# AER-RC/RRTMG_LW

Measured on AMD Instinct MI355X. Metric: columns/sec, 72-layer profiles, higher is better.
Workload: dtype f64 (transmittance / tfn codes and their LDS table f32); 1 GPU; 1000000 synthetic 72-layer columns, config 'cloudy' (icld=2: rtrnmr max-random overlap, idrv=0), sharded 1x1000000; ncol_total=1000000, nlay=72, columns_per_gpu=1000000, parallelism=columns/1, gather=none, kdata=stand-in (real k-data absent from the reference mount), sweeps=production

## Files before the change

### include/rrtmg_lw_hip.h

```cpp
#ifndef RRTMG_LW_HIP_H
#define RRTMG_LW_HIP_H

#ifdef __cplusplus
extern "C" {
#endif

#define RRTMG_LW_HIP_OK 0
#define RRTMG_LW_HIP_EPHYSICS 1
#define RRTMG_LW_HIP_EARG 2
#define RRTMG_LW_HIP_ENODEVICE 3
#define RRTMG_LW_HIP_ENOTINIT 4
#define RRTMG_LW_HIP_EDATA 5
#define RRTMG_LW_HIP_EHIP 6

#define RRTMG_LW_NBND 16
#define RRTMG_LW_NGPT 140

int rrtmg_lw_hip_init(const char *static_tables_path, const char *kdata_path, double cpdair, int device);

int rrtmg_lw_hip_init_devices(const char *static_tables_path, const char *kdata_path, double cpdair, int ndev, const int *devices);
int rrtmg_lw_hip_num_devices(void);

int rrtmg_lw_hip_kdata_is_standin(void);

// ... 208 lines not shown
    double *uflx, double *dflx, double *hr, double *uflxc, double *dflxc, double *hrc,
    double *duflx_dt, double *duflxc_dt);
int rrtmg_lw_hip_queue_flush(void);
int rrtmg_lw_hip_queue_columns(void);

unsigned rrtmg_lw_hip_build_flags(void);
int rrtmg_lw_hip_set_batch(int ncol_batch);
int rrtmg_lw_hip_effective_batch(int nlay);
int rrtmg_lw_hip_set_overlap(int on);
int rrtmg_lw_hip_set_cu_partition(int layer_cus);
int rrtmg_lw_hip_cu_partition(void);
int rrtmg_lw_hip_set_one_sweep_max(int ncol);
int rrtmg_lw_hip_set_split_max(int ncol);
int rrtmg_lw_hip_set_graph_max(int ncol);
void rrtmg_lw_hip_graph_stats(long long *captures, long long *replays);
int rrtmg_lw_hip_set_wide_window(int on);

int rrtmg_lw_hip_set_layer_split(int on);
int rrtmg_lw_hip_set_column_sort(int on, int min_gain);
int rrtmg_lw_hip_column_sort_min(void);
int rrtmg_lw_hip_set_column_sort_clear(int percent);
int rrtmg_lw_hip_column_sort_clear(void);
int rrtmg_lw_hip_set_clear_groups(int on);
long long rrtmg_lw_hip_workspace_bytes(void);
int rrtmg_lw_hip_set_n1_prototype(int on);
int rrtmg_lw_hip_n1_prototype(void);
int rrtmg_lw_hip_num_chunks(void);
int rrtmg_lw_hip_gpoints(void);

void rrtmg_lw_hip_profile_begin(void);
int rrtmg_lw_hip_profile_end(char *buf, int len);

int rrtmg_lw_hip_host_register(void *ptr, long long bytes);
int rrtmg_lw_hip_host_unregister(void *ptr);
int rrtmg_lw_hip_host_is_registered(const void *ptr, long long bytes);
int rrtmg_lw_hip_host_static(const void *ptr, long long bytes);
int rrtmg_lw_hip_host_changed(const void *ptr, int keep);
void rrtmg_lw_hip_combine_stats(long long *calls, long long *passes);

int rrtmg_lw_hip_gas_optics(int ncol, int nlay, int idrv,
    const double *play, const double *plev, const double *tlay, const double *tlev, const double *tsfc,
    const double *h2ovmr, const double *o3vmr, const double *co2vmr, const double *ch4vmr, const double *n2ovmr,
    const double *o2vmr, const double *cfc11vmr, const double *cfc12vmr, const double *cfc22vmr,
    const double *ccl4vmr, const double *emis,
    double *taug, double *fracs, double *planklay, double *planklev, double *plankbnd, double *dplankbnd_dt);
int rrtmg_lw_hip_gas_optics_device(int ncol, int nlay, int idrv,
// ... 174 lines not shown
```

### rrtmg_lw_amd/api.py

```python
from __future__ import annotations

import ctypes as C
import os

import numpy as np

_HERE = os.path.dirname(os.path.abspath(__file__))
LIB_PATH = os.environ.get("RRTMG_LW_HIP_LIB", os.path.join(_HERE, "librrtmg_lw_hip.so"))
STATIC_BLOB = os.path.join(_HERE, "data", "lw_static.bin")
STANDIN_KDATA = os.path.join(_HERE, "data", "standin.kdata.bin")
REAL_KDATA = os.path.join(os.path.dirname(_HERE), "data", "rrtmg_lw.kdata.bin")
NBND, NGPT = 16, 140

LIB_PATH_G256 = os.path.join(_HERE, "librrtmg_lw_hip_g256.so")

_dp = C.POINTER(C.c_double)
_lib = None
_libs = {}
_gpoints = 140
_initialised = False


class RrtmgLwError(RuntimeError):
    pass
# ... 164 lines not shown

def set_wide_window(on):
    return int(lib().rrtmg_lw_hip_set_wide_window(C.c_int(1 if on else 0)))


def set_column_sort(on, min_gain=-1):
    return int(lib().rrtmg_lw_hip_set_column_sort(C.c_int(1 if on else 0), C.c_int(int(min_gain))))


def column_sort_min():
    return int(lib().rrtmg_lw_hip_column_sort_min())


def set_column_sort_clear(percent):
    return int(lib().rrtmg_lw_hip_set_column_sort_clear(C.c_int(int(percent))))


def column_sort_clear():
    return int(lib().rrtmg_lw_hip_column_sort_clear())


def set_clear_groups(on):
    return int(lib().rrtmg_lw_hip_set_clear_groups(C.c_int(1 if on else 0)))


def cu_partition():
    return int(lib().rrtmg_lw_hip_cu_partition())


def _f(a, shape, dtype=np.float64):
    a = np.asfortranarray(a, dtype=dtype)
    if tuple(a.shape) != tuple(shape):
        raise ValueError(f"array has shape {a.shape}, interface declares {shape}")
    return a


def _p(a):
    return a.ctypes.data_as(_dp)


def _out_ok(a, shape, name, dtype=np.float64):
    if not (isinstance(a, np.ndarray) and a.dtype == dtype and a.flags.f_contiguous and a.flags.writeable and tuple(a.shape) == tuple(shape)):
        raise ValueError(f"output array {name!r} must be a writeable {np.dtype(dtype).name} Fortran-ordered array of shape {tuple(shape)}")
    return a


# ... 758 lines not shown
```

### rrtmg_lw_amd/csrc/driver.hip

```cpp
#include <hip/hip_runtime.h>
#include <cstdlib>
#include <sched.h>

#include <algorithm>
#include <array>
#include <atomic>
#include <cstdint>
#include <cstdarg>
#include <mutex>
#include <string>
#include <chrono>
#include <condition_variable>
#include <functional>
#include <map>
#include <thread>
#include <type_traits>
#include <vector>

#include "../../include/rrtmg_lw_hip.h"
#include "kernels.hip"
#include "mtjump.hpp"
#include "hostrows.hpp"
#include "owned.hpp"

// ... 542 lines not shown
        const State::PrepSet &ps = G.prep[0];
        W.percol = ps.percol; W.laytrop = ps.laytrop; W.ncbands = ps.ncbands; W.cflag = ps.cflag;
        W.odcld = ps.odcld; W.efcl = ps.efcl; W.ovl = ps.ovl;
        W.btop = ps.btop; W.order = ps.order; W.hgrp = ps.hgrp; W.hblk = ps.hblk; W.bbot = ps.bbot; W.hbot = ps.hbot;
    }
    G.ws = State::WsShape{nlay, ncolb, cloud, mc, want_gdp, want_efcl, want_ovl, two_scr, ng, slabcols};
    return 0;
}

int ensure_mask(int nlay, size_t ncol)
{
    const size_t bytes = (size_t)KJ_NWORD * nlay * ncol * sizeof(unsigned);
    return grow(G.mask, bytes, bytes, "sub-column masks");
}

bool g_colsort = []() { const char *e = getenv("RRTMG_LW_COLSORT"); return !e || atoi(e) != 0; }();
bool use_colsort(bool gcm, int mode, int nb);
constexpr int COLSORT_NEVER = 1 << 24;
int g_colsort_min = []() { const char *e = getenv("RRTMG_LW_COLSORT_MIN"); return e ? std::max(0, std::min(atoi(e), COLSORT_NEVER)) : 24; }();
constexpr int COLSORT_CLEAR_MAX = 1000;
constexpr int COLSORT_CLEAR_DEFAULT = 18;
int g_colsort_clear = []() { const char *e = getenv("RRTMG_LW_COLSORT_CLEAR"); return e ? std::max(0, std::min(atoi(e), COLSORT_CLEAR_MAX)) : COLSORT_CLEAR_DEFAULT; }();
bool g_clear_groups = []() { const char *e = getenv("RRTMG_LW_CLEAR_GROUPS"); return !e || atoi(e) != 0; }();

Workspace ws_for(int k, bool sorted)
{
    Workspace w = G.W;
    const State::PrepSet &ps = G.prep[k];
    w.perm = sorted ? ps.perm : nullptr;
    w.wsort = sorted ? ps.wsort : nullptr;
    w.tlayc = ps.tlayc; w.tlevc = ps.tlevc; w.cldfc = ps.cldfc;
    w.wide = ps.wide;
    w.percol = ps.percol; w.laytrop = ps.laytrop; w.ncbands = ps.ncbands; w.cflag = ps.cflag;
    w.odcld = ps.odcld; w.efcl = ps.efcl; w.ovl = ps.ovl;
    w.btop = ps.btop; w.order = ps.order; w.hgrp = ps.hgrp; w.hblk = ps.hblk; w.bbot = ps.bbot; w.hbot = ps.hbot;
    const State::ScrSet &ss = G.scrset[G.ws.two_scr ? k : 0];
    for (int a = 0; a < NSCR; a++) w.scr[a] = ss.scr[a];
    w.fw = ss.fw;
    return w;
}

int make_stream(Stream &st, int lo, int hi)
{
    if (hi <= lo) { HIP_TRY(hipStreamCreateWithFlags(st.slot(), hipStreamNonBlocking)); return 0; }
    uint32_t mask[32] = {};
    const int nw = (G.cu_total + 31) / 32;
// ... 40 lines not shown
    if (fork) HIP_TRY(hipEventRecord(G.ev_join.get(), side));
    if (scan) {
        LAUNCH("k_cloudscan", (k_cloudscan<GCM>), cgrid1, cblock1, s, Wk, g, c, b.nb, b.col0, b.nct, b.inflag, b.iceflag, b.liqflag, b.mode);
        if (fork) HIP_TRY(hipStreamWaitEvent(s, G.ev_join.get(), 0));
        const dim3 lgrid((b.nb + BLOCK - 1) / BLOCK, Wk.nlay), lblock(BLOCK);
        LAUNCH("k_cloudlay", (k_cloudlay<GCM>), lgrid, lblock, s, G.D, Wk, g, c, b.nb, b.col0, b.nct, b.mode, b.inflag, b.iceflag, b.liqflag);
        LAUNCH("k_blocksort", k_blocksort, dim3(1), dim3(256), s, Wk, (b.nb + 63) / 64, one_sweep(b.nb, b.mode) ? 1 : 0);
    }
    return launches_ok();
}

LayerArgs layer_args(const Batch &b, const double *tauaer)
{
    LayerArgs la;
    la.ncol = b.nb; la.col0 = b.col0; la.nct = b.nct; la.idrv = b.idrv; la.istart = b.istart; la.iend = b.iend;
    la.ktab_bytes = (int)(G.H.ktab.size() * 8);
    la.tauaer = tauaer;
    const unsigned gx = (b.nb + LAYER_BLOCK - 1) / LAYER_BLOCK;
    const auto bits = [](std::initializer_list<int> bands) { unsigned m = 0; for (int b : bands) m |= 1u << (b - 1); return m; };
    const unsigned quarter[4] = {bits({1, 2, 11, 15, 6}), bits({8, 10, 14, 16, 12, 13}), bits({4, 9, 7}), bits({3, 5})};
    const unsigned pairs_ = gx * (unsigned)b.nlay;
    la.nparts = !g_layer_split ? 1 : (pairs_ * 4 <= 1152 ? 4 : (pairs_ * 2 <= 1152 ? 2 : 1));
    for (int p = 0; p < 4; p++) la.partmask[p] = la.nparts == 4 ? quarter[p] : (la.nparts == 2 && p < 2 ? (quarter[2 * p] | quarter[2 * p + 1]) : 0xffffu);
    return la;
}

template <bool GCM>
int run_layer(hipStream_t s, const Workspace &Wk, const Batch &b, const GcmIn &g, const ColIn &c)
{
    const dim3 block(BLOCK);
    if (b.mode == 3) {
        const dim3 cgrid((b.nb + BLOCK - 1) / BLOCK, b.nlay);
        if (b.mc) LAUNCH("k_cloudmc<arrays>", (k_cloudmc<false>), cgrid, block, s, G.D, Wk, *b.mc, g, b.nb, b.col0, b.nct, b.inflag, b.iceflag, b.liqflag);
        else LAUNCH("k_cloudmc<mask>", (k_cloudmc<true>), cgrid, block, s, G.D, Wk, McIn{}, g, b.nb, b.col0, b.nct, b.inflag, b.iceflag, b.liqflag);
        LAUNCH("k_blocksort", k_blocksort, dim3(1), dim3(256), s, Wk, (b.nb + 63) / 64, one_sweep(b.nb, b.mode) ? 1 : 0);
    }
    const LayerArgs la = layer_args(b, GCM ? g.tauaer : c.taua);
    const unsigned gx = (b.nb + LAYER_BLOCK - 1) / LAYER_BLOCK;
    const dim3 lgrid(gx, b.nlay, la.nparts), lblock(LAYER_BLOCK);
    Workspace Wn = Wk;
    if (!GCM || !HAVE_WIDE || !g_wide_window) Wn.wide = nullptr;
    const dim3 wgrid(gx * b.nlay, la.nparts);
    if (Wn.wide) HIP_TRY(hipMemsetAsync(Wn.wide, 0, sizeof(int), s));
    if (b.share != 0) {
        if constexpr (GCM && !TUNING) {
            if (b.mode != 3 || b.mc || !Wk.odg) return fail(RRTMG_LW_HIP_EARG, "internal: shared gas optics without the mask or the optical-depth array");
            if (b.share == 1) {
                LAUNCH("k_layer<mcshare,0>", (k_layer<true, CL_SHARE, 0>), lgrid, lblock, s, G.D, Wn, g, c, la);
                if (Wn.wide) LAUNCH("k_layer<mcshare,1>", (k_layer<true, CL_SHARE, 1>), wgrid, lblock, s, G.D, Wn, g, c, la);
            } else {
                LAUNCH("k_codet", k_codet, dim3((b.nb + BLOCK - 1) / BLOCK, b.nlay), block, s, G.D, Wk, b.nb, b.col0);
            }
            return launches_ok();
        } else return fail(RRTMG_LW_HIP_EARG, "shared gas optics: GCM entries only");
    }
    const int cloud = b.mode == 0 ? 0 : b.mode == 3 ? (b.mc ? 2 : 3) : 1;
    if (TUNING && !GCM) return fail(RRTMG_LW_HIP_EARG, "tuning build: GCM entry only");
    if (TUNING && cloud != 1) return fail(RRTMG_LW_HIP_EARG, "tuning build: cloudy non-McICA calls only");
    static const char *const names[4][2] = {{"k_layer<clear,0>", "k_layer<clear,1>"}, {"k_layer<cloud,0>", "k_layer<cloud,1>"},
                                            {"k_layer<mcica,0>", "k_layer<mcica,1>"}, {"k_layer<mcmask,0>", "k_layer<mcmask,1>"}};
    if (int rc = with_const<0, 1, 2, 3>(cloud, [&](auto CL) {
            constexpr int cl = decltype(CL)::value;
// ... 140 lines not shown
    const size_t b_pc = align_up((size_t)NPERCOL * n * 8, 256), b_lt = align_up(n * 4, 256);
    const size_t b_wide = align_up((2 + ((n + LAYER_BLOCK - 1) / LAYER_BLOCK) * L) * 4, 256);
    if (int rc = grow(G.opt_buf, b_pc + b_lt + b_wide, b_pc + b_lt + b_wide, "gas-optics workspace")) return rc;
    G.opt_percol = G.opt_buf.as<double>();
    G.opt_laytrop = (int *)(G.opt_buf.as<char>() + b_pc);
    G.opt_wide = (int *)(G.opt_buf.as<char>() + b_pc + b_lt);
    HIP_TRY(hipMemset(G.opt_wide, 0, 8));
    G.opt_nlay = nlay;
    G.opt_ncolb = ncolb;
    return 0;
}

template <bool GCM>
int run_optics(hipStream_t s, const Batch &b, const GcmIn &g, const ColIn &c, const OptOut &o)
{
    Workspace W{};
    W.ncolb = G.opt_ncolb; W.pcb = G.opt_ncolb; W.nlay = b.nlay; W.err = G.d_err.as<int>();
    W.percol = G.opt_percol; W.laytrop = G.opt_laytrop;
    W.wide = GCM && HAVE_WIDE && g_wide_window ? G.opt_wide : nullptr;
    LAUNCH("k_colprep", (k_colprep<GCM>), dim3((b.nb + 63) / 64), dim3(64), s, G.D, W, g, c, b.nb, b.col0, b.nct, b.idrv, 1, 0);
    const LayerArgs la = layer_args(b, nullptr);
    const unsigned gx = (b.nb + LAYER_BLOCK - 1) / LAYER_BLOCK;
    if (W.wide) HIP_TRY(hipMemsetAsync(W.wide, 0, sizeof(int), s));
    LAUNCH("k_optics", (k_optics<GCM, 0>), dim3(gx, b.nlay, la.nparts), dim3(LAYER_BLOCK), s, G.D, W, g, c, la, o);
    if constexpr (GCM && HAVE_WIDE) {
        if (W.wide) LAUNCH("k_optics<wide>", (k_optics<true, 1>), dim3(gx * b.nlay, la.nparts), dim3(LAYER_BLOCK), s, G.D, W, g, c, la, o);
    }
    return launches_ok();
}

int check_optics(int idrv, const OptOut &o)
{
    if (!o.taug || !o.fracs) return fail(RRTMG_LW_HIP_EARG, "gas optics: taug and fracs are required");
    if (idrv == 1 && !o.dplankbnd) return fail(RRTMG_LW_HIP_EARG, "gas optics: idrv=1 needs dplankbnd_dt");
    return 0;
}

int ensure_pipeline()
{
    if (G.aux) return 0;
    Event *const ev[] = {&G.ev_in, &G.ev_last, &G.ev_fork, &G.ev_join, &G.ev_ready[0], &G.ev_layer[0], &G.ev_done[0], &G.ev_ready[1], &G.ev_layer[1], &G.ev_done[1]};
    int rc = 0;
    for (Event *e : ev) if (rc == 0) rc = make_event(*e);
    if (rc == 0) rc = make_stream(G.aux, 0, 0);
    if (rc != 0) for (Event *e : ev) (void)e->reset();
    return rc;
}
// ... 22 lines not shown
    const McIn *const mc = call.mc;
    const int nbmax = balanced_batch(ncol, eff_batch(nlay));
    const bool single = ncol <= nbmax && !(G.split_sweep && G.cu_layer > 0);
    const hipStream_t aux = single ? s : G.aux.get();
    ColIn c{};
    const bool split = G.split_sweep && G.ws.two_scr && !(mode == 3 && mc);
    const bool part = split && G.cu_layer > 0;
    if (part && !G.lay_m) {
        if (int rc = make_stream(G.lay_u, 0, 0)) return rc;
        if (int rc = make_stream(G.lay_m, 0, G.cu_layer)) return rc;
    }
    if (G.ev_last_valid) HIP_TRY(hipStreamWaitEvent(s, G.ev_last.get(), 0));
    State::GraphEnt *gent = nullptr;
    bool capture = false;
    if (single && !split && !gen.on && !mc && !G.profile && !G.n1 && ncol <= g_graph_max) {
        std::vector<unsigned char> key;
        key_put(key, ncol); key_put(key, call.nct); key_put(key, nlay); key_put(key, mode); key_put(key, idrv); key_put(key, call.inflag); key_put(key, call.iceflag); key_put(key, call.liqflag);
        const double *gp[] = {g.play, g.plev, g.tlay, g.tlev, g.tsfc, g.h2ovmr, g.o3vmr, g.co2vmr, g.ch4vmr, g.n2ovmr, g.o2vmr, g.cfc11vmr, g.cfc12vmr,
                              g.cfc22vmr, g.ccl4vmr, g.emis, g.cldfr, g.taucld, g.cicewp, g.cliqwp, g.reice, g.reliq, g.tauaer, g.tauctot,
                              out.uflx, out.dflx, out.hr, out.uflxc, out.dflxc, out.hrc, out.duflx_dt, out.duflxc_dt, out.fnet, out.fnetc,
                              out.uflxs, out.dflxs, out.uflxcs, out.dflxcs, out.uflx_var, out.dflx_var, out.hr_var};
        key_put(key, gp);
        key_put(key, G.init_gen); key_put(key, G.device);
        key_put(key, G.ws_buf.get()); key_put(key, G.ws_buf.bytes()); key_put(key, g_colsort); key_put(key, g_colsort_min); key_put(key, g_colsort_clear); key_put(key, g_clear_groups); key_put(key, g_one_sweep_max);
        key_put(key, g_wide_window); key_put(key, g_layer_split); key_put(key, g_prep_fork); key_put(key, G.sweep_fanout); key_put(key, eff_batch(nlay)); key_put(key, g_split_max);
        for (auto &e : G.graphs) if (e.key == key) { gent = &e; break; }
        if (!gent) {
            if (G.graphs.size() >= GRAPH_CACHE) {
                size_t old = 0;
                for (size_t j = 1; j < G.graphs.size(); j++) if (G.graphs[j].used < G.graphs[old].used) old = j;
                G.graphs.erase(G.graphs.begin() + (long)old);
            }
            G.graphs.emplace_back();
            gent = &G.graphs.back();
            gent->key = key;
        }
        gent->used = ++G.graph_clock;
        if (gent->exec) {
            HIP_TRY(hipGraphLaunch(gent->exec.get(), s));
            G.graph_replays++;
            HIP_TRY(hipEventRecord(G.ev_last.get(), s));
            G.ev_last_valid = true;
            return 0;
        }
        capture = gent->seen >= 1 && !gent->failed;
        gent->seen++;
        if (capture && !G.cap) { if (int rc = make_stream(G.cap, 0, 0)) return rc; }
// ... 1228 lines not shown
}

int rrtmg_lw_hip_set_column_sort_clear(int percent)
{
    ENTRY_LOCK;
    const int prev = g_colsort_clear;
    g_colsort_clear = std::max(0, std::min(percent, COLSORT_CLEAR_MAX));
    return prev;
}
int rrtmg_lw_hip_column_sort_clear(void)
{
    ENTRY_LOCK;
    return g_colsort_clear;
}

int rrtmg_lw_hip_set_clear_groups(int on)
{
    ENTRY_LOCK;
    const int prev = g_clear_groups ? 1 : 0;
    g_clear_groups = on != 0;
    return prev;
}

int rrtmg_lw_hip_set_cu_partition(int layer_cus)
{
    ENTRY_LOCK;
    if (!G.init) return fail(RRTMG_LW_HIP_ENOTINIT, "rrtmg_lw_hip_init has not been called");
    State *const keep = g_cur;
    int rc = 0;
    for (int d = 0; d < g_ndev && rc == 0; d++) {
        g_cur = &g_states[d];
        (void)hipSetDevice(G.device);
        (void)hipDeviceSynchronize();
        int n = layer_cus <= 0 ? 0 : std::max(8, std::min(G.cu_total - 8, (layer_cus + 4) / 8 * 8));
        if (G.cu_total < 16) n = 0;
        G.swset[1] = {};
        G.lay_u.reset();
        G.lay_m.reset();
        G.cu_layer = n;
        if (n > 0) {
            G.split_sweep = true;
            if ((rc = make_stream(G.lay_u, 0, 0)) == 0 && (rc = make_stream(G.lay_m, 0, n)) == 0) rc = ensure_sweep_set(1);
            if (rc != 0 && d > 0) g_states[0].err = G.err;
        }
    }
    g_cur = keep;
// ... 2091 lines not shown
```

### rrtmg_lw_amd/csrc/kernels.hip

```cpp
#include <hip/hip_runtime.h>
#include "kissjump.hpp"

#ifdef RRLW_TUNE
#define RRLW_BF_TUNE 1u
#else
#define RRLW_BF_TUNE 0u
#endif
#ifdef RRLW_G256
#define RRLW_BF_G256 8u
#else
#define RRLW_BF_G256 0u
#endif
#if defined(RRLW_LAYER_BLOCK) || defined(RRLW_STAGE_DOUBLES) || defined(RRLW_LAYER_WAVES) || defined(RRLW_LOAD_CHUNK) || defined(RRLW_MINOR_WIN) || \
    defined(RRLW_COLSORT_WIN) || defined(RRLW_SWEEPC_P0) || defined(RRLW_SWEEPC_P2D) || defined(RRLW_SWEEPC_WAVES_CAP) || defined(RRLW_SWEEPC_CODES) || \
    defined(RRLW_SWEEPZ_WAVES_G1) || defined(RRLW_SWEEPZ_WAVES_IDRV) || defined(RRLW_LAYER_STAMPS) || \
    defined(RRLW_DBG_DUMP)
#define RRLW_BF_GEOMETRY 16u
#else
#define RRLW_BF_GEOMETRY 0u
#endif

#include <algorithm>
#include <type_traits>
#include <utility>
// ... 3 lines not shown
namespace rrlw {

constexpr unsigned BUILD_FLAGS = RRLW_BF_TUNE | RRLW_BF_G256 | RRLW_BF_GEOMETRY;

struct DevTables {
    const double *ktab;
    const double *stat;
    BandLayout band[NBND];
    StaticLayout sl;
    double absice0[2], abscld1, absliq0;
    double delwave[NBND];
    double refrat[NBND][6];
    double heatfac, fluxfac, oneminus, bpade;
};

enum Field {
    F_FAC00, F_FAC01, F_FAC10, F_FAC11,
    F_COLH2O, F_COLCO2, F_COLO3, F_COLN2O, F_COLCO, F_COLCH4, F_COLO2, F_COLBRD,
    F_COLDRY, F_SELFFAC, F_SELFFRAC, F_FORFAC, F_FORFRAC, F_MINORFRAC, F_SCALEMINOR, F_SCALEMINORN2,
    F_PAVEL, F_WX1, F_WX2, F_WX3, F_WX4,
    NFIELD
};
enum PerCol { PC_PLANKBND = 0, PC_DPLANKBND = 16, PC_SECDIFF = 32, NPERCOL = 48 };
enum Scr { S_CODE, S_CODET, NSCR };
struct alignas(16) Part2 { double a, b; };

typedef float scr_t;
constexpr int CODE_WORDS = 4;
constexpr int CODE_BYTES = 4 * CODE_WORDS;

struct Workspace {
    int ncolb;
    int nlay;
    double *percol;
    int *laytrop;
    int *ncbands;
    double *odcld;
    double *efcl;
    int *cflag;
    double2 *ovl;
    int *btop;
    int *order;
    int *hgrp;
    int *hblk;
    int *bbot;
    int *hbot;
// ... 578 lines not shown
    R1(K_BINARY, H2O, CO2, R_H2OCO2, true, true, 0, false, 0, {NOM, NOM, NOM}, 0, {0, 0}, C_NONE, 0),
    ZERO_REGION)
BAND_TRAITS(13, 4,
    R1(K_BINARY, H2O, N2O, R_H2ON2O, true, true, 0, false, 2,
       {{A_ADJ, CO2, true, 2, 3.0, 2.0, 0.68, 3.55e-4}, {A_COL, CO, true, 4, 0, 0, 0, 0}, NOM}, 0, {0, 0}, C_NONE, 0),
    R1(K_NONE, 0, 0, 0, false, false, -1, false, 1, {{A_COL, O3, false, 0, 0, 0, 0, 0}, NOM, NOM}, 0, {0, 0}, C_NONE, 0))
BAND_TRAITS(14, 2,
    R1(K_SINGLE, CO2, 0, 0, true, true, -1, false, 0, {NOM, NOM, NOM}, 0, {0, 0}, C_NONE, 0),
    R1(K_SINGLE, CO2, 0, 0, false, false, -1, false, 0, {NOM, NOM, NOM}, 0, {0, 0}, C_NONE, 0))
BAND_TRAITS(15, 2,
    R1(K_BINARY, N2O, CO2, R_N2OCO2, true, true, 0, false, 1, {{A_BRD, BRD, true, 2, 0, 0, 0, 0}, NOM, NOM}, 0, {0, 0}, C_NONE, 0),
    ZERO_REGION)
BAND_TRAITS(16, 2,
    R1(K_BINARY, H2O, CH4, R_H2OCH4, true, true, 0, false, 0, {NOM, NOM, NOM}, 0, {0, 0}, C_NONE, 0),
    R1(K_SINGLE, CH4, 0, 0, false, false, -1, false, 0, {NOM, NOM, NOM}, 0, {0, 0}, C_NONE, 0))
#undef R1

__device__ const double kMult4[16] = {1, 1, 1, 1, 1, 1, 1, 0.92, 0.88, 1.07, 1.1, 0.99, 0.88, 0.943, 1, 1};
__device__ const double kMult7[16] = {1, 1, 1, 1, 1, 0.92, 0.88, 1.07, 1.1, 0.99, 0.855, 1, 1, 1, 1, 1};

struct LayerCoef {
    double f[NFIELD];
    int jp, jt, jt1, indself, indfor, indminor;
};

struct Spec { double speccomb, specparm, fs; int js; };
__device__ __forceinline__ Spec spec_calc(double cola, double rat, double colb, double mult, double oneminus)
{
    Spec s;
    s.speccomb = cola + rat * colb;
    s.specparm = fdiv(cola, s.speccomb);
    if (s.specparm >= oneminus) s.specparm = oneminus;
    const double specmult = mult * s.specparm;
    s.js = 1 + (int)specmult;
    s.fs = specmult - (double)(int)specmult;
    return s;
}

__device__ __forceinline__ void stencil6(double specparm, double fs, double fa, double fb, int &off, double (&w)[6])
{
    if (specparm < 0.125) {
        const double p = fs - 1, p2 = p * p, p4 = p2 * p2;
        const double fk0 = p4, fk1 = 1 - p - 2.0 * p4, fk2 = p + p4;
        off = 0;
        w[0] = fk0 * fa; w[1] = fk1 * fa; w[2] = fk2 * fa; w[3] = fk0 * fb; w[4] = fk1 * fb; w[5] = fk2 * fb;
    } else if (specparm > 0.875) {
// ... 33 lines not shown
#ifdef RRLW_G256
__host__ __device__ constexpr int band_ng(int B) { return B >= 1 ? 16 : 16; }
#else
__host__ __device__ constexpr int band_ng(int B) { return B == 1 ? 10 : B == 2 ? 12 : B == 3 ? 16 : B == 4 ? 14 : B == 5 ? 16 : B == 6 ? 8 : B == 7 ? 12 :
                                                    B == 8 ? 8 : B == 9 ? 12 : B == 10 ? 6 : B == 11 ? 8 : B == 12 ? 8 : B == 13 ? 4 : 2; }
#endif
__host__ __device__ constexpr int band_nquad(int B) { return (band_ng(B) + 3) / 4; }
__host__ __device__ constexpr int band_qstart(int B)
{
    int s = 0;
    for (int b = 1; b < B; b++) s += band_nquad(b);
    return s;
}
constexpr int NQUAD = band_qstart(17);
__host__ __device__ constexpr int band_g0(int B)
{
    int s = 0;
    for (int b = 1; b < B; b++) s += band_ng(b);
    return s;
}
static_assert(band_g0(17) == NGPT, "g-point table");
static_assert(NQUAD == (NGPT == 140 ? 38 : 64), "quad table");

constexpr int NRATCHI = 6 * 59 + 7 * 59;
__shared__ double s_ratchi[NRATCHI];

template <int N>
struct Rows {
    unsigned off[N > 0 ? N : 1];
    double w[N > 0 ? N : 1];
    unsigned fw;
};

template <int B> constexpr unsigned lo_binary_mask() { return (BT<B>::lo.key == K_BINARY ? 1u << (B - 1) : 0u) | lo_binary_mask<B - 1>(); }
template <> constexpr unsigned lo_binary_mask<0>() { return 0u; }
template <int B> constexpr unsigned up_binary_mask() { return (BT<B>::up.key == K_BINARY ? 1u << (B - 1) : 0u) | up_binary_mask<B - 1>(); }
template <> constexpr unsigned up_binary_mask<0>() { return 0u; }
template <int B> constexpr unsigned up_zero_mask() { return (BT<B>::up.key == K_ZERO ? 1u << (B - 1) : 0u) | up_zero_mask<B - 1>(); }
template <> constexpr unsigned up_zero_mask<0>() { return 0u; }
template <int B> constexpr unsigned up_from_a_mask() { return (BT<B>::up.frac_from_a ? 1u << (B - 1) : 0u) | up_from_a_mask<B - 1>(); }
template <> constexpr unsigned up_from_a_mask<0>() { return 0u; }
constexpr unsigned LO_BINARY = lo_binary_mask<16>(), UP_BINARY = up_binary_mask<16>(), UP_ZERO = up_zero_mask<16>(), UP_FROM_A = up_from_a_mask<16>();
static_assert((UP_BINARY & ~LO_BINARY) == 0u, "fw slots are assigned by the lower region");
__host__ __device__ constexpr int popcnt_c(unsigned v) { int n = 0; for (; v; v &= v - 1) n++; return n; }
constexpr int NFW = popcnt_c(LO_BINARY);
__host__ __device__ constexpr int fw_slot(int B) { return popcnt_c(LO_BINARY & ((1u << (B - 1)) - 1u)); }

template <int B, bool LOWER, int N, int IM>
__device__ __forceinline__ void rows_prep_minor(const DevTables &T, const LayerCoef &C, Rows<N> &rw)
{
    constexpr Region R = LOWER ? BT<B>::lo : BT<B>::up;
    constexpr unsigned ng = BT<B>::ng;
    constexpr Minor M = R.m[IM];
    constexpr int I0 = region_minor_base(R, LOWER, IM);
    const BandLayout &L = T.band[B - 1];
    const double mf = C.f[F_MINORFRAC];
    double amount;
    if constexpr (M.amt == A_COL) amount = C.f[F_COLH2O + M.sp];
    else if constexpr (M.amt == A_BRD_N2) amount = C.f[F_COLBRD] * C.f[F_SCALEMINORN2];
    else if constexpr (M.amt == A_O2) amount = C.f[F_COLO2] * C.f[F_SCALEMINOR];
    else if constexpr (M.amt == A_BRD) amount = C.f[F_COLBRD] * C.f[F_SCALEMINOR];
    else {
        const double colx = C.f[F_COLH2O + M.sp], coldry = C.f[F_COLDRY];
        const double chiref = M.chiconst > 0. ? M.chiconst : s_ratchi[(T.sl.chi - T.sl.rat) + M.sp * 59 + C.jp];
        const double chi = fdiv(colx, coldry);
        const double ratx = fdiv(1.e20 * chi, chiref);
        amount = colx;
        if (ratx > M.thr) amount = (M.base + pow(ratx - M.base, M.expo)) * chiref * coldry * 1.e-20;
    }
    const unsigned slot = (unsigned)(LOWER ? L.minor_lo[IM] : L.minor_up[IM]);
    if constexpr (M.two_d) {
        constexpr unsigned nj = LOWER ? 9 : 5;
        const Spec sm = spec_calc(C.f[F_COLH2O + R.a], T.refrat[B - 1][M.refslot], C.f[F_COLH2O + R.b], LOWER ? 8. : 4., T.oneminus);
        const unsigned r = slot + ((unsigned)(C.indminor - 1) * nj + (unsigned)(sm.js - 1)) * ng;
        rw.off[I0] = r;                    rw.w[I0] = amount * ((1. - mf) * (1. - sm.fs));
        rw.off[I0 + 1] = r + ng;           rw.w[I0 + 1] = amount * ((1. - mf) * sm.fs);
        rw.off[I0 + 2] = r + nj * ng;      rw.w[I0 + 2] = amount * (mf * (1. - sm.fs));
        rw.off[I0 + 3] = r + nj * ng + ng; rw.w[I0 + 3] = amount * (mf * sm.fs);
    } else {
        const unsigned r = slot + (unsigned)(C.indminor - 1) * ng;
        rw.off[I0] = r;          rw.w[I0] = amount * (1. - mf);
        rw.off[I0 + 1] = r + ng; rw.w[I0 + 1] = amount * mf;
    }
}

template <int B, bool LOWER, int N>
__device__ __forceinline__ void rows_prep(const DevTables &T, const LayerCoef &C, Rows<N> &rw)
{
    constexpr Region R = LOWER ? BT<B>::lo : BT<B>::up;
    constexpr unsigned ng = BT<B>::ng;
    const BandLayout &L = T.band[B - 1];
    const int jp = C.jp, jt = C.jt, jt1 = C.jt1;
    const double *rat_tab = s_ratchi;
    rw.fw = 0u;
    if constexpr (R.key == K_ZERO) return;

    double corradj = 1.;
    if constexpr (R.corr == C_B1LO) { if (C.f[F_PAVEL] < 250.) corradj = 1. - 0.15 * (250. - C.f[F_PAVEL]) / 154.4; }
    else if constexpr (R.corr == C_B1UP) corradj = 1. - 0.15 * (C.f[F_PAVEL] / 95.6);
    else if constexpr (R.corr == C_B2LO) corradj = 1. - .05 * (C.f[F_PAVEL] - 100.) / 900.;

    if constexpr (R.key == K_SINGLE) {
        const unsigned r0 = LOWER ? ((jp - 1) * 5 + (jt - 1)) : ((jp - 13) * 5 + (jt - 1));
        const unsigned r1 = LOWER ? (jp * 5 + (jt1 - 1)) : ((jp - 12) * 5 + (jt1 - 1));
        const unsigned tab = (unsigned)(LOWER ? L.absa : L.absb);
        const double colk = C.f[F_COLH2O + R.a];
        rw.off[0] = tab + r0 * ng;       rw.w[0] = colk * C.f[F_FAC00];
        rw.off[1] = tab + (r0 + 1) * ng; rw.w[1] = colk * C.f[F_FAC10];
        rw.off[2] = tab + r1 * ng;       rw.w[2] = colk * C.f[F_FAC01];
        rw.off[3] = tab + (r1 + 1) * ng; rw.w[3] = colk * C.f[F_FAC11];
    } else if constexpr (R.key == K_BINARY) {
        const double cola = C.f[F_COLH2O + R.a], colb = C.f[F_COLH2O + R.b];
        const double rat = rat_tab[R.rat * 59 + (jp - 1)], rat_1 = rat_tab[R.rat * 59 + jp];
        constexpr double mult = LOWER ? 8. : 4.;
        const Spec s = spec_calc(cola, rat, colb, mult, T.oneminus);
        const Spec s1 = spec_calc(cola, rat_1, colb, mult, T.oneminus);
        if constexpr (LOWER) {
            const unsigned tab = (unsigned)L.absa;
            const int ind0 = ((jp - 1) * 5 + (jt - 1)) * 9 + s.js - 1;
            const int ind1 = (jp * 5 + (jt1 - 1)) * 9 + s1.js - 1;
            int so;
            double w6[6];
            stencil6(s.specparm, s.fs, C.f[F_FAC00], C.f[F_FAC10], so, w6);
            unsigned r = tab + (unsigned)(ind0 + so) * ng;
            rw.off[0] = r;           rw.w[0] = s.speccomb * w6[0];
            rw.off[1] = r + ng;      rw.w[1] = s.speccomb * w6[1];
            rw.off[2] = r + 2 * ng;  rw.w[2] = s.speccomb * w6[2];
            rw.off[3] = r + 9 * ng;  rw.w[3] = s.speccomb * w6[3];
            rw.off[4] = r + 10 * ng; rw.w[4] = s.speccomb * w6[4];
            rw.off[5] = r + 11 * ng; rw.w[5] = s.speccomb * w6[5];
            stencil6(s1.specparm, s1.fs, C.f[F_FAC01], C.f[F_FAC11], so, w6);
            r = tab + (unsigned)(ind1 + so) * ng;
            rw.off[6] = r;            rw.w[6] = s1.speccomb * w6[0];
            rw.off[7] = r + ng;       rw.w[7] = s1.speccomb * w6[1];
            rw.off[8] = r + 2 * ng;   rw.w[8] = s1.speccomb * w6[2];
            rw.off[9] = r + 9 * ng;   rw.w[9] = s1.speccomb * w6[3];
// ... 289 lines not shown
    constexpr int NP = 4 * band_nquad(B);
    constexpr bool SCALED = BL::R.mult != 0;
#pragma unroll
    for (int j = 0; j < NP; j++) tau[j] = (SCALED || j >= BL::ng) ? 0.0 : tau0;
    if constexpr (BL::NL > 0) {
        double2 b0[BL::CH], b1[BL::CH];
        BL::template issue<0, LDS>(kt, lds, rw, b0);
        BL::template step<0, LDS>(kt, lds, rw, b0, b1, tau);
    }
    if constexpr (SCALED) {
#pragma unroll
        for (int j = 0; j < BL::ng; j++) {
            if constexpr (BL::R.mult == 4) tau[j] = fma(tau[j], kMult4[j], tau0);
            else if constexpr (BL::R.mult == 7) tau[j] = fma(tau[j], kMult7[j], tau0);
        }
    }
}

struct LayerArgs {
    int ncol, col0, nct, idrv, istart, iend;
    int nparts;
    unsigned partmask[4];
    int ktab_bytes;
    const double *tauaer;
};

struct alignas(16) scr4 { scr_t v[4]; };

typedef float scr_vec __attribute__((ext_vector_type(4)));
struct pk4 { unsigned w[CODE_WORDS]; };
__device__ __forceinline__ pk4 pack4(const scr4 &v)
{
    pk4 p;
#pragma unroll
    for (int k = 0; k < 4; k++) p.w[k] = __float_as_uint(v.v[k]);
    return p;
}
__device__ __forceinline__ scr4 unpack4(const pk4 &p)
{
    scr4 v;
#pragma unroll
    for (int k = 0; k < 4; k++) v.v[k] = __uint_as_float(p.w[k]);
    return v;
}
typedef unsigned pk_vec __attribute__((ext_vector_type(CODE_WORDS)));
__device__ __forceinline__ void scr_store(unsigned *base, size_t cell, const scr4 &v)
// ... 267 lines not shown
        }
    }
}

#ifndef RRLW_LAYER_WAVES
#define RRLW_LAYER_WAVES 3
#endif

struct LayerWg { double2 *lds; int jp0, im0, tid, nth, pc; bool lower, ok; };

template <int B, int CLOUD, class WN, int BASE_LO, int BASE_UP>
__device__ __forceinline__ void layer_band(const DevTables &T, const Workspace &W, const LayerArgs &a, const LayerCoef &C,
                                           __amdgpu_buffer_rsrc_t kt, const LayerWg &wg, bool lower, int lay, int col, bool incol, int cloudy,
                                           const unsigned (&mw)[MASK_WORDS])
{
    STAMP(4);
    unsigned delta[NROLE];
#pragma unroll
    for (int r = 0; r < NROLE; r++) delta[r] = 0u;
    const bool use_lds = __builtin_amdgcn_ballot_w64(!wg.ok) == 0ull;
    const size_t ncb = W.ncolb, gcx = (size_t)a.col0 + wg.pc;
    double odcld = 0.0;
    if constexpr (CLOUD == 1 || CLOUD == 3 || CLOUD == CL_SHARE) { if (cloudy) odcld = W.odcld[((size_t)(B - 1) * W.nlay + (lay - 1)) * ncb + col]; }
    const double secdiff = W.percol[(size_t)(PC_SECDIFF + B - 1) * ncb + col];
    const double taua = col_load(a.tauaer + (size_t)a.col0 + (size_t)a.nct * ((lay - 1) + (size_t)W.nlay * (B - 1)), (unsigned)wg.pc * 8u);
    unsigned gbits = 0u;
    if constexpr (CLOUD == 3 || CLOUD == CL_SHARE) {
        (void)mw;
        constexpr int g0 = band_g0(B), ng = BT<B>::ng, w0 = g0 >> 5, w1 = (g0 + ng - 1) >> 5;
        if (cloudy) {
            const unsigned *mrow = W.mask + (size_t)(lay - 1) * W.mask_stride + W.mask_col0 + gcx;
            const unsigned long long lo = mrow[(size_t)w0 * W.nlay * W.mask_stride];
            const unsigned long long hi = w1 != w0 ? mrow[(size_t)w1 * W.nlay * W.mask_stride] : 0u;
            gbits = (unsigned)(((lo | (hi << 32)) >> (g0 & 31)) & ((1ull << ng) - 1ull));
        }
    }
    if (lower) {
        constexpr int N = region_nrows(BT<B>::lo, true);
        Rows<N> rw;
        rows_prep<B, true, N>(T, C, rw);
        if (use_lds) {
            band_delta<B, true, WN, BASE_LO>(T, wg.jp0, wg.im0, delta);
            rows_to_lds<B, true, N>(rw, delta);
            STAMP(2);
            band_cells<B, CLOUD, true, N, true>(T, W, kt, wg.lds, rw, lay, col, incol, secdiff, taua, cloudy, odcld, gbits);
        } else {
            band_cells<B, CLOUD, true, N, false>(T, W, kt, wg.lds, rw, lay, col, incol, secdiff, taua, cloudy, odcld, gbits);
// ... 201 lines not shown
        const double tz_up = GCM ? col_load(g.tlev + ro + nct, o8) : c.tz[gc + (size_t)nct * lay];
        const double tz_lo = lay == 1 ? (GCM ? col_load(g.tlev + ro, o8) : c.tz[gc]) : 0.0;
        for (int b = 0; b < NBND; b++) {
            if (!((bmask >> b) & 1u)) continue;
            const double *tp = S + T.sl.totplnk + 181 * b;
            if (o.planklay) opt_store(o.planklay + ro + (size_t)nct * nlv * b, bytes, off8, planck_band(tp, tavel));
            if (o.planklev) {
                const size_t lv0 = (size_t)a.col0 + (size_t)nct * (nlv + 1) * b;
                opt_store(o.planklev + lv0 + (size_t)nct * lay, bytes, off8, planck_band(tp, tz_up));
                if (lay == 1) opt_store(o.planklev + lv0, bytes, off8, planck_band(tp, tz_lo));
            }
            if (lay == 1) {
                if (o.plankbnd) opt_store(o.plankbnd + a.col0 + (size_t)nct * b, bytes, off8, W.percol[(size_t)(PC_PLANKBND + b) * W.ncolb + col]);
                if (o.dplankbnd && a.idrv == 1) opt_store(o.dplankbnd + a.col0 + (size_t)nct * b, bytes, off8, W.percol[(size_t)(PC_DPLANKBND + b) * W.ncolb + col]);
            }
        }
    }
    const __amdgpu_buffer_rsrc_t kt = __builtin_amdgcn_make_buffer_rsrc((void *)T.ktab, 0, a.ktab_bytes, 0x00020000);
    const unsigned mw[MASK_WORDS] = {};
#ifdef RRLW_LAYER_STAMPS
    if ((threadIdx.x & 63) == 0) { for (int i = 0; i < NSTAMP; i++) s_stamp[(threadIdx.x >> 6) * (NSTAMP + 1) + i] = 0ull; }
    STAMP(-1);
#endif
    for (int i = threadIdx.x; i < NRATCHI; i += LAYER_BLOCK) s_ratchi[i] = S[T.sl.rat + i];
    if (!early) {
        if (threadIdx.x == 0) { s_wg[0] = lower ? 1 : 0; s_wg[1] = 99; s_wg[2] = 99; s_wg[3] = 0; s_wg[4] = 0; }
        __syncthreads();
    }
    LayerWg wg;
    wg.lds = s_tab; wg.tid = threadIdx.x; wg.nth = blockDim.x; wg.pc = pc;
    wg.lower = s_wg[0] != 0;
    if (!early) {
        const bool in = lower == wg.lower;
        int jlo = in ? jp : 99, ilo = in ? indminor : 99, jhi = in ? jp : 0, ihi = in ? indminor : 0;
#pragma unroll
        for (int o = 32; o >= 1; o >>= 1) {
            jlo = min(jlo, __shfl_xor(jlo, o, 64)); ilo = min(ilo, __shfl_xor(ilo, o, 64));
            jhi = max(jhi, __shfl_xor(jhi, o, 64)); ihi = max(ihi, __shfl_xor(ihi, o, 64));
        }
        if ((threadIdx.x & 63) == 0) { atomicMin(&s_wg[1], jlo); atomicMin(&s_wg[2], ilo); atomicMax(&s_wg[3], jhi); atomicMax(&s_wg[4], ihi); }
    }
    __syncthreads();
    wg.jp0 = s_wg[1];
    using WN = std::conditional_t<WIDE != 0, WinWide, WinNarrow>;
    wg.im0 = min(s_wg[2], 20 - WN::MW);
    wg.ok = lower == wg.lower && (unsigned)(jp - wg.jp0) <= (unsigned)(WN::NPL - 2) && (unsigned)(indminor - wg.im0) <= (unsigned)(WN::MW - 2);
    STAMP(5);
    passes_run<CLOUD, WN>(static_cast<std::conditional_t<WIDE != 0, LayerPassesWide, LayerPasses> *>(nullptr), T, W, a, C, kt, wg, lower, lay, col, incol, cloudy, mw, bmask, o);
#ifdef RRLW_LAYER_STAMPS
    STAMP(4);
    if ((threadIdx.x & 63) == 0) {
        for (int i = 0; i < NSTAMP; i++) atomicAdd(&g_stamps[i], s_stamp[(threadIdx.x >> 6) * (NSTAMP + 1) + i]);
        atomicAdd(&g_stamps[NSTAMP], 1ull);
    }
#endif
}

template <bool GCM, int CLOUD, int WIDE>
__device__ __forceinline__ void layer_grid(const DevTables &T, const Workspace &W, const GcmIn &g, const ColIn &c, const LayerArgs &a, double2 *s_tab, int *s_wg,
                                           const OptOut &o)
{
    const int part = WIDE == 0 ? blockIdx.z : blockIdx.y;
    unsigned bmask = ((a.iend >= 32 ? 0u : (1u << a.iend)) - 1u) & ~((1u << (a.istart - 1)) - 1u);
    if (a.nparts > 1) bmask &= a.partmask[part];
    if constexpr (WIDE == 0) {
        layer_cells<GCM, CLOUD, 0>(T, W, g, c, a, s_tab, s_wg, blockIdx.x, blockIdx.y, bmask, part == 0, o);
    } else {
        const int n = __builtin_amdgcn_readfirstlane(W.wide[0]), gx = (a.ncol + LAYER_BLOCK - 1) / LAYER_BLOCK;
        if ((int)blockIdx.x >= n) return;
        const int item = __builtin_amdgcn_readfirstlane(W.wide[2 + blockIdx.x]);
        layer_cells<GCM, CLOUD, 1>(T, W, g, c, a, s_tab, s_wg, item % gx, item / gx, bmask, false, o);
    }
}
template <bool GCM, int CLOUD, int WIDE>
__global__ __launch_bounds__(LAYER_BLOCK, RRLW_LAYER_WAVES) void k_layer(DevTables T, Workspace W, GcmIn g, ColIn c, LayerArgs a)
{
    __shared__ double2 s_tab[STAGE_DOUBLES / 2];
    __shared__ int s_wg[5];
    layer_grid<GCM, CLOUD, WIDE>(T, W, g, c, a, s_tab, s_wg, OptOut{});
}
template <bool GCM, int WIDE>
__global__ __launch_bounds__(LAYER_BLOCK, RRLW_LAYER_WAVES) void k_optics(DevTables T, Workspace W, GcmIn g, ColIn c, LayerArgs a, OptOut o)
{
    __shared__ double2 s_tab[STAGE_DOUBLES / 2];
    __shared__ int s_wg[5];
    layer_grid<GCM, CL_OPTICS, WIDE>(T, W, g, c, a, s_tab, s_wg, o);
}

__global__ __launch_bounds__(256) void k_codet(DevTables T, Workspace W, int ncol, int col0)
// ... 95 lines not shown
        const double factor = (radice - 2.) / 3.;
        index_i = (int)factor; if (index_i == 43) index_i = 42;
        fint_i = factor - (double)index_i;
        index_i = clampi(index_i, 1, 42);
    } else if (iceflag == 3) {
        if (radice < 5.0 || radice > 140.0) ice_err = E_ICE_GEN_BOUNDS;
        const double factor = (radice - 2.) / 3.;
        index_i = (int)factor; if (index_i == 46) index_i = 45;
        fint_i = factor - (double)index_i;
        index_i = clampi(index_i, 1, 45);
    }
    if (liqflag == 1) {
        if (radliq < 2.5 || radliq > 60.) liq_err = E_LIQ_BOUNDS;
        index_l = (int)(radliq - 1.5);
        if (index_l == 0) index_l = 1;
        if (index_l == 58) index_l = 57;
        fint_l = radliq - 1.5 - (double)index_l;
        index_l = clampi(index_l, 1, 57);
    }
    int err = 0, any = 0, quad = 0;
#pragma unroll 1
    for (int B = 1; B <= NBND; B++) {
        const int ng = band_ng(B), g0 = band_g0(B);
        const double secdiff = W.percol[(size_t)(PC_SECDIFF + B - 1) * ncb + col];
        double ai = 0.0, al = 0.0;
        if (inflag == 2) {
            if (iceflag == 0) ai = T.absice0[0] + T.absice0[1] / radice;
            else if (iceflag == 1) {
                const int icx = B <= 2 ? B : (B <= 5 ? 3 : (B <= 8 ? 4 : 5));
                ai = absice1[2 * (icx - 1)] + absice1[2 * (icx - 1) + 1] / radice;
            } else if (iceflag == 2) { const double *t = absice2 + 43 * (B - 1); ai = t[index_i - 1] + fint_i * (t[index_i] - t[index_i - 1]); }
            else if (iceflag == 3) { const double *t = absice3 + 46 * (B - 1); ai = t[index_i - 1] + fint_i * (t[index_i] - t[index_i - 1]); }
            if (liqflag == 0) al = T.absliq0;
            else if (liqflag == 1) { const double *t = absliq1 + 58 * (B - 1); al = t[index_l - 1] + fint_l * (t[index_l] - t[index_l - 1]); }
        }
        const double tband = FROMMASK ? g.taucld[(B - 1) + (size_t)NBND * cl] : 0.0;
        if constexpr (FROMMASK) {
            const unsigned long long lo = mw[g0 >> 5], hi = (g0 >> 5) < MASK_WORDS - 1 ? mw[(g0 >> 5) + 1] : 0u;
            const unsigned bits = (unsigned)(((lo | (hi << 32)) >> (g0 & 31)) & ((1ull << ng) - 1ull));
            double t = tband, od = 0.0, ef = 0.0;
            if (bits) {
                if (mciwp + mclwp >= cldmin || t >= cldmin) {
                    if (inflag == 1) err = E_MC_INFLAG1;
                    else if (inflag == 2) {
                        double a_i = 0.0, a_l = 0.0;
                        if (mciwp != 0.0 && iceflag >= 0 && iceflag <= 3) { a_i = ai; if (ice_err && !err) err = ice_err; }
                        if (mclwp != 0.0) {
// ... 2529 lines not shown
```

Before: 18.20 million columns/s.

## Shrink ratchi LDS staging to a jp window and fold constant secdiff bands

After: 17.79 million columns/s. 0.978x the previous value.

```diff
diff --git a/include/rrtmg_lw_hip.h b/include/rrtmg_lw_hip.h
--- a/include/rrtmg_lw_hip.h
+++ b/include/rrtmg_lw_hip.h
@@ -254,6 +254,7 @@
 int rrtmg_lw_hip_set_column_sort_clear(int percent);
 int rrtmg_lw_hip_column_sort_clear(void);
 int rrtmg_lw_hip_set_clear_groups(int on);
+int rrtmg_lw_hip_set_layer_order(int order);
 long long rrtmg_lw_hip_workspace_bytes(void);
 int rrtmg_lw_hip_set_n1_prototype(int on);
 int rrtmg_lw_hip_n1_prototype(void);
diff --git a/rrtmg_lw_amd/api.py b/rrtmg_lw_amd/api.py
--- a/rrtmg_lw_amd/api.py
+++ b/rrtmg_lw_amd/api.py
@@ -210,6 +210,10 @@
 
 def set_clear_groups(on):
     return int(lib().rrtmg_lw_hip_set_clear_groups(C.c_int(1 if on else 0)))
+
+
+def set_layer_order(order):
+    return int(lib().rrtmg_lw_hip_set_layer_order(C.c_int(1 if order else 0)))
 
 
 def cu_partition():
diff --git a/rrtmg_lw_amd/csrc/driver.hip b/rrtmg_lw_amd/csrc/driver.hip
--- a/rrtmg_lw_amd/csrc/driver.hip
+++ b/rrtmg_lw_amd/csrc/driver.hip
@@ -588,6 +588,8 @@
 constexpr int COLSORT_CLEAR_DEFAULT = 18;
 int g_colsort_clear = []() { const char *e = getenv("RRTMG_LW_COLSORT_CLEAR"); return e ? std::max(0, std::min(atoi(e), COLSORT_CLEAR_MAX)) : COLSORT_CLEAR_DEFAULT; }();
 bool g_clear_groups = []() { const char *e = getenv("RRTMG_LW_CLEAR_GROUPS"); return !e || atoi(e) != 0; }();
+constexpr int LAYER_ORDER_DEFAULT = 0;
+int g_layer_order = []() { const char *e = getenv("RRTMG_LW_LAYER_ORDER"); return e ? (atoi(e) != 0 ? 1 : 0) : LAYER_ORDER_DEFAULT; }();
 
 Workspace ws_for(int k, bool sorted)
 {
@@ -674,7 +676,13 @@
     const unsigned pairs_ = gx * (unsigned)b.nlay;
     la.nparts = !g_layer_split ? 1 : (pairs_ * 4 <= 1152 ? 4 : (pairs_ * 2 <= 1152 ? 2 : 1));
     for (int p = 0; p < 4; p++) la.partmask[p] = la.nparts == 4 ? quarter[p] : (la.nparts == 2 && p < 2 ? (quarter[2 * p] | quarter[2 * p + 1]) : 0xffffu);
+    la.order = g_layer_order != 0 && gx <= 65535u ? 1 : 0;
     return la;
+}
+dim3 layer_grid_dim(const LayerArgs &la, int nlay)
+{
+    const unsigned gx = (la.ncol + LAYER_BLOCK - 1) / LAYER_BLOCK;
+    return la.order ? dim3((unsigned)nlay, gx, la.nparts) : dim3(gx, (unsigned)nlay, la.nparts);
 }
 
 template <bool GCM>
@@ -689,7 +697,7 @@
     }
     const LayerArgs la = layer_args(b, GCM ? g.tauaer : c.taua);
     const unsigned gx = (b.nb + LAYER_BLOCK - 1) / LAYER_BLOCK;
-    const dim3 lgrid(gx, b.nlay, la.nparts), lblock(LAYER_BLOCK);
+    const dim3 lgrid = layer_grid_dim(la, b.nlay), lblock(LAYER_BLOCK);
     Workspace Wn = Wk;
     if (!GCM || !HAVE_WIDE || !g_wide_window) Wn.wide = nullptr;
     const dim3 wgrid(gx * b.nlay, la.nparts);
@@ -876,7 +884,7 @@
     const LayerArgs la = layer_args(b, nullptr);
     const unsigned gx = (b.nb + LAYER_BLOCK - 1) / LAYER_BLOCK;
     if (W.wide) HIP_TRY(hipMemsetAsync(W.wide, 0, sizeof(int), s));
-    LAUNCH("k_optics", (k_optics<GCM, 0>), dim3(gx, b.nlay, la.nparts), dim3(LAYER_BLOCK), s, G.D, W, g, c, la, o);
+    LAUNCH("k_optics", (k_optics<GCM, 0>), layer_grid_dim(la, b.nlay), dim3(LAYER_BLOCK), s, G.D, W, g, c, la, o);
     if constexpr (GCM && HAVE_WIDE) {
         if (W.wide) LAUNCH("k_optics<wide>", (k_optics<true, 1>), dim3(gx * b.nlay, la.nparts), dim3(LAYER_BLOCK), s, G.D, W, g, c, la, o);
     }
@@ -945,7 +953,7 @@
                               out.uflxs, out.dflxs, out.uflxcs, out.dflxcs, out.uflx_var, out.dflx_var, out.hr_var};
         key_put(key, gp);
         key_put(key, G.init_gen); key_put(key, G.device);
-        key_put(key, G.ws_buf.get()); key_put(key, G.ws_buf.bytes()); key_put(key, g_colsort); key_put(key, g_colsort_min); key_put(key, g_colsort_clear); key_put(key, g_clear_groups); key_put(key, g_one_sweep_max);
+        key_put(key, G.ws_buf.get()); key_put(key, G.ws_buf.bytes()); key_put(key, g_colsort); key_put(key, g_colsort_min); key_put(key, g_colsort_clear); key_put(key, g_clear_groups); key_put(key, g_layer_order); key_put(key, g_one_sweep_max);
         key_put(key, g_wide_window); key_put(key, g_layer_split); key_put(key, g_prep_fork); key_put(key, G.sweep_fanout); key_put(key, eff_batch(nlay)); key_put(key, g_split_max);
         for (auto &e : G.graphs) if (e.key == key) { gent = &e; break; }
         if (!gent) {
@@ -2220,6 +2228,14 @@
     return prev;
 }
 
+int rrtmg_lw_hip_set_layer_order(int order)
+{
+    ENTRY_LOCK;
+    const int prev = g_layer_order;
+    g_layer_order = order != 0 ? 1 : 0;
+    return prev;
+}
+
 int rrtmg_lw_hip_set_cu_partition(int layer_cus)
 {
     ENTRY_LOCK;
diff --git a/rrtmg_lw_amd/csrc/kernels.hip b/rrtmg_lw_amd/csrc/kernels.hip
--- a/rrtmg_lw_amd/csrc/kernels.hip
+++ b/rrtmg_lw_amd/csrc/kernels.hip
@@ -49,6 +49,8 @@
     NFIELD
 };
 enum PerCol { PC_PLANKBND = 0, PC_DPLANKBND = 16, PC_SECDIFF = 32, NPERCOL = 48 };
+__host__ __device__ constexpr bool secdiff_fixed(int B) { return B == 1 || B == 4 || B >= 10; }
+constexpr double SECDIFF_FIXED = 1.66;
 enum Scr { S_CODE, S_CODET, NSCR };
 struct alignas(16) Part2 { double a, b; };
 
@@ -673,6 +675,7 @@
 struct LayerCoef {
     double f[NFIELD];
     int jp, jt, jt1, indself, indfor, indminor;
+    int jp0, jspan;
 };
 
 struct Spec { double speccomb, specparm, fs; int js; };
@@ -752,8 +755,13 @@
 static_assert(band_g0(17) == NGPT, "g-point table");
 static_assert(NQUAD == (NGPT == 140 ? 38 : 64), "quad table");
 
-constexpr int NRATCHI = 6 * 59 + 7 * 59;
-__shared__ double s_ratchi[NRATCHI];
+constexpr int NRATCHI_TAB = 6 + 7, RATCHI_PITCH = 5;
+__shared__ double s_ratchi[NRATCHI_TAB * RATCHI_PITCH];
+__device__ __forceinline__ double ratchi(const DevTables &T, const LayerCoef &C, int tab, int d)
+{
+    const unsigned r = (unsigned)(C.jp - C.jp0);
+    return r <= (unsigned)C.jspan ? s_ratchi[tab * RATCHI_PITCH + r + d] : T.stat[T.sl.rat + tab * 59 + (C.jp - 1) + d];
+}
 
 template <int N>
 struct Rows {
@@ -792,7 +800,7 @@
     else if constexpr (M.amt == A_BRD) amount = C.f[F_COLBRD] * C.f[F_SCALEMINOR];
     else {
         const double colx = C.f[F_COLH2O + M.sp], coldry = C.f[F_COLDRY];
-        const double chiref = M.chiconst > 0. ? M.chiconst : s_ratchi[(T.sl.chi - T.sl.rat) + M.sp * 59 + C.jp];
+        const double chiref = M.chiconst > 0. ? M.chiconst : ratchi(T, C, 6 + M.sp, 1);
         const double chi = fdiv(colx, coldry);
         const double ratx = fdiv(1.e20 * chi, chiref);
         amount = colx;
@@ -821,7 +829,6 @@
     constexpr unsigned ng = BT<B>::ng;
     const BandLayout &L = T.band[B - 1];
     const int jp = C.jp, jt = C.jt, jt1 = C.jt1;
-    const double *rat_tab = s_ratchi;
     rw.fw = 0u;
     if constexpr (R.key == K_ZERO) return;
 
@@ -841,7 +848,7 @@
         rw.off[3] = tab + (r1 + 1) * ng; rw.w[3] = colk * C.f[F_FAC11];
     } else if constexpr (R.key == K_BINARY) {
         const double cola = C.f[F_COLH2O + R.a], colb = C.f[F_COLH2O + R.b];
-        const double rat = rat_tab[R.rat * 59 + (jp - 1)], rat_1 = rat_tab[R.rat * 59 + jp];
+        const double rat = ratchi(T, C, R.rat, 0), rat_1 = ratchi(T, C, R.rat, 1);
         constexpr double mult = LOWER ? 8. : 4.;
         const Spec s = spec_calc(cola, rat, colb, mult, T.oneminus);
         const Spec s1 = spec_calc(cola, rat_1, colb, mult, T.oneminus);
@@ -1177,6 +1184,7 @@
     int nparts;
     unsigned partmask[4];
     int ktab_bytes;
+    int order;
     const double *tauaer;
 };
 
@@ -1490,7 +1498,8 @@
     const size_t ncb = W.ncolb, gcx = (size_t)a.col0 + wg.pc;
     double odcld = 0.0;
     if constexpr (CLOUD == 1 || CLOUD == 3 || CLOUD == CL_SHARE) { if (cloudy) odcld = W.odcld[((size_t)(B - 1) * W.nlay + (lay - 1)) * ncb + col]; }
-    const double secdiff = W.percol[(size_t)(PC_SECDIFF + B - 1) * ncb + col];
+    double secdiff = SECDIFF_FIXED;
+    if constexpr (!secdiff_fixed(B)) secdiff = W.percol[(size_t)(PC_SECDIFF + B - 1) * ncb + col];
     const double taua = col_load(a.tauaer + (size_t)a.col0 + (size_t)a.nct * ((lay - 1) + (size_t)W.nlay * (B - 1)), (unsigned)wg.pc * 8u);
     unsigned gbits = 0u;
     if constexpr (CLOUD == 3 || CLOUD == CL_SHARE) {
@@ -1738,7 +1747,6 @@
     if ((threadIdx.x & 63) == 0) { for (int i = 0; i < NSTAMP; i++) s_stamp[(threadIdx.x >> 6) * (NSTAMP + 1) + i] = 0ull; }
     STAMP(-1);
 #endif
-    for (int i = threadIdx.x; i < NRATCHI; i += LAYER_BLOCK) s_ratchi[i] = S[T.sl.rat + i];
     if (!early) {
         if (threadIdx.x == 0) { s_wg[0] = lower ? 1 : 0; s_wg[1] = 99; s_wg[2] = 99; s_wg[3] = 0; s_wg[4] = 0; }
         __syncthreads();
@@ -1761,6 +1769,12 @@
     using WN = std::conditional_t<WIDE != 0, WinWide, WinNarrow>;
     wg.im0 = min(s_wg[2], 20 - WN::MW);
     wg.ok = lower == wg.lower && (unsigned)(jp - wg.jp0) <= (unsigned)(WN::NPL - 2) && (unsigned)(indminor - wg.im0) <= (unsigned)(WN::MW - 2);
+    static_assert(WN::NPL <= RATCHI_PITCH && NRATCHI_TAB * RATCHI_PITCH <= LAYER_BLOCK, "ratio / chi window");
+    {
+        const int tab = threadIdx.x / RATCHI_PITCH, i = threadIdx.x % RATCHI_PITCH, j = wg.jp0 - 1 + i;
+        if (tab < NRATCHI_TAB && i < WN::NPL && j < 59) s_ratchi[threadIdx.x] = S[T.sl.rat + tab * 59 + j];
+    }
+    C.jp0 = __builtin_amdgcn_readfirstlane(wg.jp0); C.jspan = WN::NPL - 2;
     STAMP(5);
     passes_run<CLOUD, WN>(static_cast<std::conditional_t<WIDE != 0, LayerPassesWide, LayerPasses> *>(nullptr), T, W, a, C, kt, wg, lower, lay, col, incol, cloudy, mw, bmask, o);
 #ifdef RRLW_LAYER_STAMPS
@@ -1780,7 +1794,8 @@
     unsigned bmask = ((a.iend >= 32 ? 0u : (1u << a.iend)) - 1u) & ~((1u << (a.istart - 1)) - 1u);
     if (a.nparts > 1) bmask &= a.partmask[part];
     if constexpr (WIDE == 0) {
-        layer_cells<GCM, CLOUD, 0>(T, W, g, c, a, s_tab, s_wg, blockIdx.x, blockIdx.y, bmask, part == 0, o);
+        const int bx = a.order ? blockIdx.y : blockIdx.x, by = a.order ? blockIdx.x : blockIdx.y;
+        layer_cells<GCM, CLOUD, 0>(T, W, g, c, a, s_tab, s_wg, bx, by, bmask, part == 0, o);
     } else {
         const int n = __builtin_amdgcn_readfirstlane(W.wide[0]), gx = (a.ncol + LAYER_BLOCK - 1) / LAYER_BLOCK;
         if ((int)blockIdx.x >= n) return;
@@ -1922,7 +1937,7 @@
 #pragma unroll 1
     for (int B = 1; B <= NBND; B++) {
         const int ng = band_ng(B), g0 = band_g0(B);
-        const double secdiff = W.percol[(size_t)(PC_SECDIFF + B - 1) * ncb + col];
+        const double secdiff = secdiff_fixed(B) ? SECDIFF_FIXED : W.percol[(size_t)(PC_SECDIFF + B - 1) * ncb + col];
         double ai = 0.0, al = 0.0;
         if (inflag == 2) {
             if (iceflag == 0) ai = T.absice0[0] + T.absice0[1] / radice;
```
